# flexcompute/tidy3d

Hardware: AMD Instinct MI355X
Metric: Mcells/s on 512^3 Yee grid (higher is better)
Workload: dtype f32; 1 GPU; v0: vacuum, PEC walls, curl stencil only; 512^3 Yee cells, Ez point dipole (GaussianPulse 200 THz), random +-1e-3 initial fields; parallelism=z-slab x1, bytes_per_cell_step=72

## Files before the change

### tidy3d_amd/csrc/fdtd_fused2.hpp

```cpp
#pragma once
#include "fdtd_kernels.hpp"

namespace fdtd {

constexpr int kMaxInj = 256;
struct InjP {
  int n;
  const int* start;
  const int4* ent;
  const float* val;
  const float* val2;
  int e2_in_sweep;
  float* cap;
  const int* dstart;
  const int* dlist;
  const struct DumpBox* dboxes;
  float* dump;
};
struct DumpBox {
  int lo0, lo1, lo2, nx, ny, nz;
  int off[6];
};
constexpr int kMaxDumps = 8;
struct DampT {
// ... 93 lines not shown
        if (!fused2_instantiated(fused2_lb(W, opt), opt)) return false;
        const int rep = fused2_opt(nt, mat, mon, clip, damp, disp, src, wv, true, W);
        if (!clip && fused2_rep_word(opt) && !fused2_instantiated(fused2_lb(W, rep), rep)) return false;
      }
    }
  return true;
}
static_assert(fused2_words_instantiated(), "fused2_opt forms a word that no list of instantiations holds");

#if !defined(FDTD_NO_EXJ)
#define FDTD_NO_EXJ 0
#endif
constexpr bool fused2_exj(int lb, int opt) { return !FDTD_NO_EXJ && (opt & kF2Damp) == 0 && !(lb == 512 && (opt & kF2Mat) != 0); }
constexpr int fused2_xch_arrays(int lb, int opt) {
  const int wv = fused2_whatif(opt);
  if (wv) return wv == 13 ? 9 : ((wv >= 10 && wv <= 12) ? 6 + (wv == 11 ? 2 : 3) : 8);
  return fused2_exj(lb, opt) ? 9 : 8;
}
constexpr size_t fused2_lds_bytes(int lb, int opt, int waves) {
  return ((size_t)fused2_xch_arrays(lb, opt) * waves * 64 + ((opt & kF2Damp) ? 2 * 64 : 0)) * sizeof(float4) + ((opt & kF2Mat) ? (size_t)kMaxMedia * sizeof(float2) : 0);
}
static_assert(fused2_lds_bytes(1024, kF2NT | kF2Mat | kF2Mon | kF2Clip | kF2Disp | kF2Src, 16) <= 160 * 1024 && fused2_lds_bytes(1024, kF2Mat | kF2Damp, 16) <= 160 * 1024 &&
              2 * fused2_lds_bytes(512, kF2NT, 8) <= 160 * 1024 && 2 * fused2_lds_bytes(512, kF2Mat | kF2Damp, 8) <= 160 * 1024,
              "fused2_step_kernel: LDS of a workgroup (two per CU for eight waves)");
constexpr bool fused2_lds_pinned(int lb, int opt) {
  const int wv = fused2_whatif(opt), w = lb / 64;
  if (wv) return fused2_lds_bytes(lb, opt, 16) == ((size_t)(wv == 13 ? 9 : ((wv >= 10 && wv <= 12) ? 6 + (wv == 11 ? 2 : 3) : 8)) * 16 * 64) * sizeof(float4);
  return fused2_lds_bytes(lb, opt, w) == ((size_t)(fused2_exj(lb, opt) ? 9 : 8) * w * 64 + ((opt & 8) ? 2 * 64 : 0)) * sizeof(float4) + ((opt & 2) ? (size_t)kMaxMedia * sizeof(float2) : 0);
}
#define FDTD_F2_X(LBV, OV) && fused2_lds_pinned(LBV, OV)
static_assert(true FDTD_F2_LIST_ALL(FDTD_F2_X), "fused2_lds_bytes: the LDS of a listed instantiation changed");
#undef FDTD_F2_X
constexpr int kMaxCap = 1024;
constexpr int kSeamArrays = 13;

void launch_inject_values(hipStream_t st, float* val, const float* w_re, const float* w_im, const float2* wave,
                          long long step, int n);
struct Fused2Launch {
  hipStream_t st;
  int waves, opt, grid_blocks;
  GridP g; FieldP a, b; StepP s; MatP m;
  int zchunk, nbx, nby, nbz, xcd_remap;
  InjP inj; float* seam; DampT dmp; ClipP clip; TileClassP tcl; DispP dp; SrcP sr;
};
#define FDTD_F2_ARGS(L) (L).g, (L).a, (L).b, (L).s, (L).m, (L).zchunk, (L).nbx, (L).nby, (L).nbz, (L).xcd_remap, (L).inj, (L).seam, (L).dmp, (L).clip, (L).tcl, (L).dp, (L).sr
#define FDTD_F2_CASE(LBV, OV)                                                                                                      \
  case fused2_key(LBV, OV):                                                                                                        \
    hipLaunchKernelGGL((fused2_step_kernel<LBV, OV>), dim3(L.grid_blocks, 1, 1), dim3(64, L.waves, 1), fused2_lds_bytes(LBV, OV, L.waves), L.st, \
                       FDTD_F2_ARGS(L));                                                                                           \
    return true;
#define FDTD_F2_LAUNCHER(NAME, LIST)                                                                                               \
  bool NAME(const Fused2Launch& L) {                                                                                               \
    switch (fused2_key(fused2_lb(L.waves, L.opt), L.opt)) { LIST(FDTD_F2_CASE) default: return false; }                            \
  }
bool launch_fused2_step(const Fused2Launch& L);
bool launch_fused2_step_src(const Fused2Launch& L);
bool launch_fused2_step_whatif(const Fused2Launch& L);
bool launch_fused2_step_disp(const Fused2Launch& L);
bool launch_fused2_step_clip(const Fused2Launch& L);
void launch_inject_table(hipStream_t st, float* tab, long long stride, long long off, const float* w_re, const float* w_im,
                         const float2* wave, long long n_steps, int n);
constexpr int kPairMons = 4;
struct PairRecP {
  int n_mon;
  int pre_done;
  BoxP box[kPairMons];
  int nc[kPairMons];
  int comp[kPairMons][6];
  int cap_off[kPairMons];
  float* out_n[kPairMons];
  float* out_m[kPairMons];
};
void launch_pair_record(hipStream_t st, const PairRecP& r, long long max_cells, const GridP& g, const FieldP& a, const FieldP& b,
                        const float* cap);
struct DftDumpP { int n; int slot[3]; int off[3]; };
void launch_dft_record_dump(hipStream_t st, const DftDumpP& r, const float* dump, float2* acc, long long cells, long long fstride,
                            const float2* phase, int nf);
void launch_seams(hipStream_t st, const GridP& g, const FieldP& b, const StepP& s, const MatP& m, const float* seam,
                  int n_seams, const DampT& dmp, const ClipP& clip, const InjP& inj, const SrcP& sr = SrcP{}, float* rep = nullptr);
constexpr int kRepArraysHost = 7;
inline size_t seam_scratch_floats(const GridP& g, int n_tiles_x) { return (size_t)n_tiles_x * kSeamArrays * (size_t)(g.nz + 2) * (size_t)g.ny; }
inline size_t seam_rep_floats(const GridP& g, int n_tiles_x) { return (size_t)n_tiles_x * kRepArraysHost * (size_t)g.nz * (size_t)g.ny; }
void launch_seam_flush(hipStream_t st, const GridP& g, const FieldP& b, const float* rep, int n_seams);

}
```

### tidy3d_amd/csrc/fdtd_kernels2.hpp

```cpp
#pragma once
#include "fdtd_fused2.hpp"

namespace fdtd {

__global__ __launch_bounds__(256) void pair_record_kernel(PairRecP r, GridP g, FieldP a, FieldP b, const float* cap) {
  const int mi = blockIdx.y / 6, ic = blockIdx.y % 6;
  if (mi >= r.n_mon || ic >= r.nc[mi]) return;
  const BoxP bx = r.box[mi];
  const long long cells = (long long)bx.nx * bx.ny * bx.nz;
  const long long t = (long long)blockIdx.x * blockDim.x + threadIdx.x;
  if (t >= cells) return;
  const int c = r.comp[mi][ic];
  const int lx = (int)(t % bx.nx), ly = (int)((t / bx.nx) % bx.ny), lz = (int)(t / ((long long)bx.nx * bx.ny));
  const long long p = (long long)(bx.lo2 + lz) * g.sxy + (long long)(bx.lo1 + ly) * g.nx + bx.lo0 + lx;
  const long long idx = (long long)ic * cells + t;
  const float* fa = c == 0 ? a.ex : (c == 1 ? a.ey : (c == 2 ? a.ez : (c == 3 ? a.hx : (c == 4 ? a.hy : a.hz))));
  const float* fb = c == 0 ? b.ex : (c == 1 ? b.ey : (c == 2 ? b.ez : (c == 3 ? b.hx : (c == 4 ? b.hy : b.hz))));
  const float mid = cap[r.cap_off[mi] + idx];
  float* on = r.out_n[mi];
  float* om = r.out_m[mi];
  if (c < 3) {
    if (on && !r.pre_done) on[idx] = 1.0f * fa[p];
    if (om) om[idx] = 1.0f * mid;
  } else {
// ... 6 lines not shown
                                                              long long fstride, const float2* phase, int nf) {
  const int q = blockIdx.y;
  const long long t = (long long)blockIdx.x * blockDim.x + threadIdx.x;
  if (t >= cells || q >= r.n) return;
  const float v = dump[r.off[q] + t];
  float2* a0 = acc + (long long)r.slot[q] * cells;
  for (int k = 0; k < nf; ++k) {
    const float2 ph = phase[k];
    float2 a = a0[(long long)k * fstride + t];
    a.x += v * ph.x;
    a.y += v * ph.y;
    a0[(long long)k * fstride + t] = a;
  }
}

__global__ __launch_bounds__(256) void inject_table_kernel(float* tab, long long stride, long long off, const float* w_re,
                                                           const float* w_im, const float2* wave, long long n_steps, int n) {
  const long long g = (long long)blockIdx.x * blockDim.x + threadIdx.x;
  if (g >= n_steps * n) return;
  const long long step = g / n;
  const int t = (int)(g % n);
  const float2 a = wave[step];
  tab[step * stride + off + t] = w_re[t] * a.x - w_im[t] * a.y;
}

__global__ __launch_bounds__(256) void inject_values_kernel(float* val, const float* w_re, const float* w_im,
                                                            const float2* wave, long long step, int n) {
  const int t = threadIdx.x;
  if (t >= n) return;
  const float2 a = wave[step];
  val[t] = w_re[t] * a.x - w_im[t] * a.y;
}

__device__ __forceinline__ long long seam_at(const GridP& g, int seam, int arr, int j, int k) {
  return (((long long)seam * kSeamArrays + arr) * (g.nz + 2) + (k + 1)) * g.ny + j;
}

constexpr int kRepArrays = 7;
__device__ __forceinline__ long long rep_base(const GridP& g, int n_tiles_x) {
  return (long long)n_tiles_x * kSeamArrays * (g.nz + 2) * g.ny;
}
__device__ __forceinline__ long long rep_at(const GridP& g, int seam, int arr, int j, int k) {
  return (((long long)seam * kRepArrays + arr) * g.nz + k) * g.ny + j;
}

__device__ __forceinline__ float lane_next(float v) {
#if defined(__HIP_DEVICE_COMPILE__)
  const int x = __builtin_bit_cast(int, v);
  return __builtin_bit_cast(float, __builtin_amdgcn_update_dpp(x, x, 0x130, 0xf, 0xf, false));
#else
  return __shfl_down(v, 1);
#endif
}
__device__ __forceinline__ float lane_prev(float v) {
#if defined(__HIP_DEVICE_COMPILE__)
  const int x = __builtin_bit_cast(int, v);
  return __builtin_bit_cast(float, __builtin_amdgcn_update_dpp(x, x, 0x138, 0xf, 0xf, false));
#else
  return __shfl_up(v, 1);
#endif
}

__device__ __forceinline__ void lds_dma16(const float* base, unsigned off, float4* dst, int lane) {
#if defined(__HIP_DEVICE_COMPILE__)
  const unsigned lds_addr = __builtin_amdgcn_readfirstlane((unsigned)(size_t)dst);
  unsigned keep;
  asm volatile("s_mov_b32 %0, m0\n\ts_mov_b32 m0, %2\n\ts_nop 0\n\tglobal_load_lds_dwordx4 %1, %3\n\ts_mov_b32 m0, %0"
               : "=&s"(keep) : "v"(off), "s"(lds_addr), "s"(base) : "memory");
#else
  dst[lane] = *reinterpret_cast<const float4*>(reinterpret_cast<const char*>(base) + off);
#endif
}
__device__ __forceinline__ void lds_dma_wait() {
// ... 14 lines not shown
  return v;
}

__device__ __forceinline__ int lane_value(int v, int l) {
#if defined(__HIP_DEVICE_COMPILE__)
  return __builtin_amdgcn_readlane(v, l);
#else
  return __shfl(v, l);
#endif
}

template <int LB, int OPT>
__device__ __forceinline__ void fused2_step_tile(const GridP& g, const FieldP& a, const FieldP& b, const StepP& s, const MatP& m,
                                                 int zchunk, int nbx, int nby, int nbz, const InjP& inj,
                                                 float* __restrict__ seam, const DampT& dmp, const ClipP& clip, int t,
                                                 const DispP& dp, const SrcP& sr) {
  constexpr int V = 4;
  constexpr bool SRC = (OPT & kF2Src) != 0;
  constexpr bool NT = (OPT & kF2NT) != 0, MAT = (OPT & kF2Mat) != 0, MON = (OPT & kF2Mon) != 0;
  constexpr bool DISP = (OPT & kF2Disp) != 0;
  constexpr int WHATIF = fused2_whatif(OPT);
  constexpr int PF = (WHATIF >= 10 && WHATIF <= 12) ? WHATIF : 0;
  constexpr bool EZL = WHATIF == 15;
  constexpr bool EXJ = (WHATIF == 0 && (OPT & kF2NoExj) == 0) || WHATIF == 13 || EZL;
  constexpr bool E1S = PF != 0 || EZL;
  constexpr int XE = E1S ? 6 : 8, XZ = 7;
  [[maybe_unused]] constexpr int NPF = PF == 11 ? 2 : (PF ? 3 : 0);
  constexpr int NXCH = E1S ? 6 : 8;
  static_assert((!PF && !EZL) || (OPT & 0xff & ~kF2NT) == 0, "prefetch instantiations: the vacuum sweep only");
  constexpr bool DAMP = (OPT & kF2Damp) != 0;
  constexpr bool CLIP = (OPT & kF2Clip) != 0;
  constexpr bool REP = (OPT & kF2Rep) != 0;
  static_assert(!REP || (!CLIP && !PF && !EZL && !DISP && !SRC), "deferred seam repair: plain, materials and absorber sweeps of the whole grid");
  const bool per_x = CLIP && g.bcx0 == BC_PERIODIC;
  const int tile_y = t % nby;
  const int tile_x = (t / nby) % nbx;
  const int tile_z = t / (nby * nbx);
  HIP_DYNAMIC_SHARED(float4, xch)
  const int tx = threadIdx.x;
  const int ty = __builtin_amdgcn_readfirstlane((int)threadIdx.y);
  const int W = blockDim.y, R = W - 3;
  const int slot = W * 64;
  const int me = ty * 64 + tx;
  {
    const float4 z4 = {0.f, 0.f, 0.f, 0.f};
#pragma unroll
    for (int q = 0; q < NXCH; ++q) xch[q * slot + me] = z4;
  }
  [[maybe_unused]] float4* xdm = xch + (EXJ ? 9 : 8) * slot;
  [[maybe_unused]] float2* lut_s = reinterpret_cast<float2*>(xdm + (DAMP ? 2 * 64 : 0));
  if constexpr (MAT) {
    for (int q = me; q < m.n_media; q += slot) lut_s[q] = m.lut[q];
  }
  if constexpr (DAMP) {
    if (ty == 0) {
      const int ii = (tile_x * 64 + tx) * V;
      float4 b4 = {1.f, 1.f, 1.f, 1.f}, c4 = {1.f, 1.f, 1.f, 1.f};
      if (ii < g.nx) { b4 = *reinterpret_cast<const float4*>(dmp.fb[0] + ii); c4 = *reinterpret_cast<const float4*>(dmp.fc[0] + ii); }
      xdm[tx] = b4; xdm[64 + tx] = c4;
    }
  }
  __syncthreads();
  const float ca = m.ca1, cb = m.cb1;
  const int k0 = (CLIP ? clip.k0 : 0) + tile_z * zchunk;
  const int k1 = min(k0 + zchunk, CLIP ? clip.k1 : g.nz);
  const int kA = k0 > 0 ? k0 - 1 : 0;
// ... 74 lines not shown
    float ezx = lane_next(ezm[0]);
    if (act && (tx == 63 || last_x)) ezx = last_x ? (per_x ? a.ez[pb] : 0.f) : a.ez[pb + ux + V];
    const float ipz = s.ipz[kA - 1];
    ldf<V, true>(ho, uni(a.hx + pb), ubc);
    ldf<V, true>(hoy, uni(a.hy + pb), ubc);
    if constexpr (REP) {
      if (act && tx == 63 && !last_x) {
        const float* r = rpl + (long long)(kA - 1) * g.ny;
        hoy[V - 1] = r[0]; exm[V - 1] = r[2 * rep_arr]; eym[V - 1] = r[3 * rep_arr]; ezm[V - 1] = r[4 * rep_arr]; ezx = r[6 * rep_arr];
        if (use_jp) ezj[V - 1] = r[4 * rep_arr + 1];
      }
      if (xh) {
        const float* r = rpr + (long long)(kA - 1) * g.ny;
        eym[0] = r[5 * rep_arr]; ezm[0] = r[6 * rep_arr];
        if (use_jp) ezj[0] = r[6 * rep_arr + 1];
      }
    }
    if constexpr (DAMP) {
      const float czp = dmp.fc[2][kA - 1];
      const float4 b4 = xdm[tx], c4 = xdm[64 + tx];
      const float bx[V] = {b4.x, b4.y, b4.z, b4.w}, cx[V] = {c4.x, c4.y, c4.z, c4.w};
#pragma unroll
      for (int e = 0; e < V; ++e) { ho[e] *= bx[e] * cyv * czp; hoy[e] *= cx[e] * byv * czp; }
    }
#pragma unroll
    for (int e = 0; e < V; ++e) h1x[e] = upd_h(ho[e], ch, ezj[e] - ezm[e], ipy, eyk[e] - eym[e], ipz);
#pragma unroll
    for (int e = 0; e < V; ++e) {
      const float ez_ip = (e + 1 < V) ? ezm[(e + 1) % V] : ezx;
      h1y[e] = upd_h(hoy[e], ch, exk[e] - exm[e], ipz, ez_ip - ezm[e], ipx[e]);
    }
  }
  int cur = 0;
  const long long seam_arr = (long long)(g.nz + 2) * g.ny;
  const long long seam_row = seam_at(g, tile_x, 0, j, 0);
  struct Ld {
    float exn[V], eyn[V], ezk[V], exj[V], ezj[V], hxn[V], hyn[V], hzn[V];
    float eyx_g, ezx_g;
    float exn_m, ez_mm, ey_mm, ex_jm, hy_o, hz_o;
  };
  [[maybe_unused]] float4* pfb = xch + NXCH * slot;
  [[maybe_unused]] auto pf_issue = [&](int k) __attribute__((always_inline)) {
    if constexpr (PF != 0) {
      const long long pb = (long long)k * g.sxy + rowb;
      const long long up = (k < g.nz) ? g.sxy : 0;
      lds_dma_fence();
      if constexpr (PF == 10) {
        lds_dma16(uni(a.hx + pb), ubc, pfb + 0 * slot + ty * 64, tx);
        lds_dma16(uni(a.hy + pb), ubc, pfb + 1 * slot + ty * 64, tx);
        lds_dma16(uni(a.hz + pb), ubc, pfb + 2 * slot + ty * 64, tx);
      } else if constexpr (PF == 11) {
        lds_dma16(uni(a.ey + pb + up), ubc, pfb + 0 * slot + ty * 64, tx);
        lds_dma16(uni(a.hy + pb), ubc, pfb + 1 * slot + ty * 64, tx);
      } else {
        lds_dma16(uni(a.ex + pb + up), ubc, pfb + 0 * slot + ty * 64, tx);
        lds_dma16(uni(a.ey + pb + up), ubc, pfb + 1 * slot + ty * 64, tx);
        lds_dma16(uni(a.ez + pb), ubc, pfb + 2 * slot + ty * 64, tx);
      }
    }
  };
  [[maybe_unused]] auto pf_take = [&](int q, float (&o)[V]) __attribute__((always_inline)) {
    const float4 t4 = pfb[q * slot + me];
    o[0] = t4.x; o[1] = t4.y; o[2] = t4.z; o[3] = t4.w;
  };
  auto issue = [&](int k, Ld& L) __attribute__((always_inline)) {
    if constexpr (WHATIF == 3) {
      if (ty < 2 || ty == W - 1) {
        zero<V>(L.exn); zero<V>(L.eyn); zero<V>(L.ezk); zero<V>(L.exj); zero<V>(L.ezj); zero<V>(L.hxn); zero<V>(L.hyn); zero<V>(L.hzn);
// ... 59 lines not shown
          if (use_jp) {
            L.ezj[V - 1] = r[4 * rep_arr + 1];
            if (!EXJ || ty == W - 1 || k == kA) L.exj[V - 1] = r[2 * rep_arr + 1];
          }
        }
        if (xh) {
          const float* r = rpr + (long long)k * g.ny;
          L.ezk[0] = r[6 * rep_arr];
          if (up1) L.eyn[0] = r[5 * rep_arr + g.ny];
          if (use_jp) L.ezj[0] = r[6 * rep_arr + 1];
          if (do_e1) {
            L.exn_m = up1 ? r[2 * rep_arr + g.ny] : a.ex[pb + im + up];
            L.ez_mm = r[4 * rep_arr]; L.ey_mm = r[3 * rep_arr];
            if (use_jp) L.ex_jm = r[2 * rep_arr + 1];
            L.hy_o = r[0]; L.hz_o = r[rep_arr];
          }
        }
      }
    }
    if constexpr (PF != 0) {
      lds_dma_wait();
      if constexpr (PF == 10) { pf_take(0, L.hxn); pf_take(1, L.hyn); pf_take(2, L.hzn); }
      else if constexpr (PF == 11) { pf_take(0, L.eyn); pf_take(1, L.hyn); }
      else { pf_take(0, L.exn); pf_take(1, L.eyn); pf_take(2, L.ezk); }
    }
  };
  Ld LA, LB2;
  auto body = [&](int k, Ld& L) __attribute__((always_inline)) {
    const int txo = (MAT || DAMP) ? tx : opaque_lane(tx);
    const int i0o = (tile_x * 64 + txo) * V;
    const bool act = i0o < g.nx, last_x = i0o + V >= g.nx, first_x = i0o == 0;
    const bool xh = act && txo == 0 && (!first_x || per_x);
    [[maybe_unused]] const bool wall_x0 = first_x && !pmc_x0 && !per_x;
    const bool seam_l = (txo == 63 && !last_x) || (per_x && last_x), seam_r = txo == 0 && (tile_x > 0 || per_x);
    const long long seam_back = (tile_x > 0 ? -1 : (long long)(nbx - 1)) * kSeamArrays * seam_arr;
    const long long pb = (long long)k * g.sxy + rowb;
    const float ipz = s.ipz[k], idz = s.idz[k];
    [[maybe_unused]] float bzk = 1.f, czk = 1.f;
    if constexpr (DAMP) { bzk = dmp.fb[2][min(k, g.nz - 1)]; czk = dmp.fc[2][min(k, g.nz - 1)]; }
    int q0 = 0, q1 = 0;
    if (inj.n > 0) { q0 = inj.start[k]; q1 = inj.start[k + 1]; }
    [[maybe_unused]] int d0 = 0, d1 = 0;
    if constexpr (MON) { if (inj.dstart) { d0 = inj.dstart[k]; d1 = inj.dstart[k + 1]; } }
    float hy_m = 0.f, hz_m = 0.f;
    float (&exn)[V] = L.exn, (&eyn)[V] = L.eyn, (&ezk)[V] = L.ezk, (&exj)[V] = L.exj, (&ezj)[V] = L.ezj;
    float (&hxn)[V] = L.hxn, (&hyn)[V] = L.hyn, (&hzn)[V] = L.hzn;
    [[maybe_unused]] uint32_t rw = kBgWord;
    if constexpr (MAT) {
      if (do_e1) rw = m.roww[((long long)min(k, g.nz - 1) * g.ny + j) * nbx + tile_x];
    }
    [[maybe_unused]] int ss = -1;
    if constexpr (SRC) {
      if (do_e1 && k < g.nz) ss = sr.sseg[((long long)k * g.ny + j) * nbx + tile_x];
    }
    [[maybe_unused]] int ds = -1;
    if constexpr (DISP) {
      if (do_e1 && k < g.nz) ds = dp.dseg[((long long)k * g.ny + j) * nbx + tile_x];
    }
    if constexpr (WHATIF == 7) {
      issue(k, L);
      if (own && k > k0 && act) {
        const long long po = pb - g.sxy + i0;
        float o0[V], o1[V], o2[V];
#pragma unroll
        for (int e = 0; e < V; ++e) { o0[e] = L.exn[e] + L.exj[e]; o1[e] = L.ezk[e] + L.ezj[e]; o2[e] = L.eyn[e]; }
        stv_h<V, NT>(b.ex + po, o0); stv_h<V, NT>(b.ey + po, o2); stv_h<V, NT>(b.ez + po, o1);
        stv_h<V, NT>(b.hx + po, L.hxn); stv_h<V, NT>(b.hy + po, L.hyn); stv_h<V, NT>(b.hz + po, L.hzn);
      }
// ... 195 lines not shown
                  hit &= hit - 1;
                  const int d = lane_value(ev.x, l) - i0, c = lane_value(ev.z, l) - 8, w = lane_value(ev.w, l);
#pragma unroll
                  for (int e = 0; e < V; ++e)
                    if (d == e) inj.cap[w] = c == 0 ? e1xn[e] : (c == 1 ? e1yn[e] : e1zn[e]);
                }
              }
            }
          }
        }
        if constexpr (MON) {
          if (own && k >= k0 && k < k1) {
            for (int q = d0; q < d1; ++q) {
              const DumpBox bx = inj.dboxes[inj.dlist[q]];
              const int ly = j - bx.lo1, lz = k - bx.lo2;
              if (ly >= 0 && ly < bx.ny) {
                const long long rowo = ((long long)lz * bx.ny + ly) * bx.nx;
#pragma unroll
                for (int e = 0; e < V; ++e) {
                  const int lx = i0o + e - bx.lo0;
                  if (lx >= 0 && lx < bx.nx && act && (!CLIP || (i0o + e >= clip.i0 && i0o + e < clip.i1))) {
                    if (bx.off[0] >= 0) inj.dump[bx.off[0] + rowo + lx] = e1xn[e];
                    if (bx.off[1] >= 0) inj.dump[bx.off[1] + rowo + lx] = e1yn[e];
                    if (bx.off[2] >= 0) inj.dump[bx.off[2] + rowo + lx] = e1zn[e];
                    if (bx.off[3] >= 0) inj.dump[bx.off[3] + rowo + lx] = hxn[e];
                    if (bx.off[4] >= 0) inj.dump[bx.off[4] + rowo + lx] = hyn[e];
                    if (bx.off[5] >= 0) inj.dump[bx.off[5] + rowo + lx] = hzn[e];
                  }
                }
              }
            }
          }
        }
        if (WHATIF != 9 && (CLIP || (own && k >= k0 && k < k1)) && act) {
          float* sp = seam + seam_row + (long long)k * g.ny;
          if (seam_l) {
            sp[0] = hyn[V - 1];
            sp[seam_arr] = hzn[V - 1];
            sp[2 * seam_arr] = e1xn[V - 1];
            sp[3 * seam_arr] = e1yn[V - 1];
            sp[4 * seam_arr] = e1zn[V - 1];
          }
          if (seam_r) {
            sp[5 * seam_arr + seam_back] = e1yn[0];
            sp[6 * seam_arr + seam_back] = e1zn[0];
          }
        }
      }
    }
    float h2x[V], h2y[V], h2z[V];
    unspecified<V>(h2x); unspecified<V>(h2y); unspecified<V>(h2z);
    if (do_h2 && k > kA) {
      if constexpr (DAMP) {
        {
          const float4 b4 = xdm[tx];
          const float bx[V] = {b4.x, b4.y, b4.z, b4.w};
#pragma unroll
          for (int e = 0; e < V; ++e) h1x[e] *= bx[e] * cyv * cz_m;
        }
        {
          const float4 c4 = xdm[64 + tx];
          const float cx[V] = {c4.x, c4.y, c4.z, c4.w};
#pragma unroll
          for (int e = 0; e < V; ++e) { h1y[e] *= cx[e] * byv * cz_m; h1z[e] *= cx[e] * cyv * bz_m; }
        }
      }
      if constexpr (SRC) {
        if (ss_m >= 0 && act && sr.t->use_h2) {
          const long long qs = ((long long)ss_m * 3) * 256 + tx * V;
          float tx_[V], ty_[V], tz_[V];
          ldv<V>(tx_, sr.t->h2 + qs); ldv<V>(ty_, sr.t->h2 + qs + 256); ldv<V>(tz_, sr.t->h2 + qs + 512);
#pragma unroll
          for (int e = 0; e < V; ++e) { h1x[e] = h1x[e] + tx_[e]; h1y[e] = h1y[e] + ty_[e]; h1z[e] = h1z[e] + tz_[e]; }
          if (sr.t->h2b) {
            ldv<V>(tx_, sr.t->h2b + qs); ldv<V>(ty_, sr.t->h2b + qs + 256); ldv<V>(tz_, sr.t->h2b + qs + 512);
#pragma unroll
            for (int e = 0; e < V; ++e) { h1x[e] = h1x[e] + tx_[e]; h1y[e] = h1y[e] + ty_[e]; h1z[e] = h1z[e] + tz_[e]; }
          }
        }
// ... 9 lines not shown
              hit &= hit - 1;
              const int d = lane_value(ev.x, l) - i0o, code = lane_value(ev.z, l);
              const float v = inj.val2[lane_value(ev.w, l)];
#pragma unroll
              for (int e = 0; e < V; ++e) {
                const bool mine = d == e;
                h1x[e] = (mine && code == 3) ? h1x[e] + v : h1x[e];
                h1y[e] = (mine && code == 4) ? h1y[e] + v : h1y[e];
                h1z[e] = (mine && code == 5) ? h1z[e] + v : h1z[e];
              }
            }
          }
        }
      }
      float eyx = lane_next(e1y[0]);
      float ezx = lane_next(e1z[0]);
      if (txo == 63 || last_x) { eyx = 0.f; ezx = 0.f; }
      float4 t0, t1;
      if constexpr (WHATIF == 6) {
        t0 = make_float4(e1x[0], e1x[1], e1x[2], e1x[3]); t1 = make_float4(e1z[0], e1z[1], e1z[2], e1z[3]);
      } else {
        t0 = xch[(4 + (E1S ? 0 : (cur ^ 1) * 2) + 0) * slot + me + 64];
        t1 = xch[(4 + (E1S ? 0 : (cur ^ 1) * 2) + 1) * slot + me + 64];
      }
      const float exj1[V] = {t0.x, t0.y, t0.z, t0.w}, ezj1[V] = {t1.x, t1.y, t1.z, t1.w};
#pragma unroll
      for (int e = 0; e < V; ++e) {
        const float ey_ip = (e + 1 < V) ? e1y[(e + 1) % V] : eyx;
        const float ez_ip = (e + 1 < V) ? e1z[(e + 1) % V] : ezx;
        h2x[e] = upd_h(h1x[e], ch, ezj1[e] - e1z[e], ipy, e1yn[e] - e1y[e], ipz_m);
        h2y[e] = upd_h(h1y[e], ch, e1xn[e] - e1x[e], ipz_m, ez_ip - e1z[e], ipx[e]);
        h2z[e] = upd_h(h1z[e], ch, ey_ip - e1y[e], ipx[e], exj1[e] - e1x[e], ipy);
      }
      if constexpr (CLIP) {
        if (act) {
          float* sq = seam + seam_row + (long long)(k - 1) * g.ny;
          if (seam_l) {
            sq[7 * seam_arr] = h2x[V - 1];
            sq[8 * seam_arr] = h2y[V - 2];
            sq[9 * seam_arr] = h2z[V - 2];
          }
          if (seam_r) {
            sq[10 * seam_arr + seam_back] = h2x[0];
            sq[11 * seam_arr + seam_back] = h2y[0];
            sq[12 * seam_arr + seam_back] = h2z[0];
          }
        }
      }
    }
    if constexpr (WHATIF != 6) {
      float4 t4;
      if constexpr (!E1S) {
        t4.x = e1xn[0]; t4.y = e1xn[1]; t4.z = e1xn[2]; t4.w = e1xn[3];
        xch[(4 + cur * 2 + 0) * slot + me] = t4;
        t4.x = e1zn[0]; t4.y = e1zn[1]; t4.z = e1zn[2]; t4.w = e1zn[3];
        xch[(4 + cur * 2 + 1) * slot + me] = t4;
      }
      if constexpr (EXJ) {
        t4.x = exn[0]; t4.y = exn[1]; t4.z = exn[2]; t4.w = exn[3];
        xch[XE * slot + me] = t4;
      }
      if constexpr (EZL) {
        if (k + 1 <= k1) {
          t4.x = ezn_pre[0]; t4.y = ezn_pre[1]; t4.z = ezn_pre[2]; t4.w = ezn_pre[3];
          xch[XZ * slot + me] = t4;
        }
      }
      t4.x = h2x[0]; t4.y = h2x[1]; t4.z = h2x[2]; t4.w = h2x[3];
      xch[2 * slot + me] = t4;
      t4.x = h2z[0]; t4.y = h2z[1]; t4.z = h2z[2]; t4.w = h2z[3];
      xch[3 * slot + me] = t4;
    }
    if constexpr (WHATIF != 2 && WHATIF != 6 && WHATIF != 8) __syncthreads();
    if constexpr (E1S) {
      float4 t4;
      t4.x = e1xn[0]; t4.y = e1xn[1]; t4.z = e1xn[2]; t4.w = e1xn[3];
      xch[4 * slot + me] = t4;
      t4.x = e1zn[0]; t4.y = e1zn[1]; t4.z = e1zn[2]; t4.w = e1zn[3];
      xch[5 * slot + me] = t4;
// ... 76 lines not shown
          while (hit) {
            const int l = __ffsll(hit) - 1;
            hit &= hit - 1;
            const int d = lane_value(ev.x, l) - i0, code = lane_value(ev.z, l);
            const float v = inj.val2[lane_value(ev.w, l)];
#pragma unroll
            for (int e = 0; e < V; ++e) {
              if (d == e) {
                if (code == 0) ex[e] += v;
                else if (code == 1) ey[e] += v;
                else ez[e] += v;
              }
            }
          }
        }
      }
      if constexpr (DAMP) {
        if (dmp.e2) {
          {
            const float4 c4 = xdm[64 + tx];
            const float cx[V] = {c4.x, c4.y, c4.z, c4.w};
#pragma unroll
            for (int e = 0; e < V; ++e) ex[e] *= cx[e] * byv * bz_m;
          }
          {
            const float4 b4 = xdm[tx];
            const float bx[V] = {b4.x, b4.y, b4.z, b4.w};
#pragma unroll
            for (int e = 0; e < V; ++e) { ey[e] *= bx[e] * cyv * bz_m; ez[e] *= bx[e] * byv * cz_m; }
          }
        }
      }
      if (act && (!CLIP || (i0o >= clip.i0 && i0o < clip.i1))) {
        float* sq = seam + seam_row + (long long)(k - 1) * g.ny;
        if (!CLIP && WHATIF != 9 && txo == 63 && !last_x) {
          sq[7 * seam_arr] = h2x[V - 1];
          sq[8 * seam_arr] = h2y[V - 2];
          sq[9 * seam_arr] = h2z[V - 2];
        }
        if (!CLIP && WHATIF != 9 && txo == 0 && tile_x > 0) {
          sq[10 * seam_arr - kSeamArrays * seam_arr] = h2x[0];
          sq[11 * seam_arr - kSeamArrays * seam_arr] = h2y[0];
          sq[12 * seam_arr - kSeamArrays * seam_arr] = h2z[0];
        }
        const long long po = pb - g.sxy + i0;
        if (WHATIF != 5 || ex[0] == 3.0e38f) {
          stv_h<V, NT>(b.hx + po, h2x);
          stv_h<V, NT>(b.hy + po, h2y);
          stv_h<V, NT>(b.hz + po, h2z);
          stv_h<V, NT>(b.ex + po, ex);
          stv_h<V, NT>(b.ey + po, ey);
          stv_h<V, NT>(b.ez + po, ez);
        }
      }
    }
#pragma unroll
    for (int e = 0; e < V; ++e) {
      h2xm[e] = h2x[e]; h2ym[e] = h2y[e];
      h1x[e] = hxn[e]; h1y[e] = hyn[e]; h1z[e] = hzn[e];
      e1x[e] = e1xn[e]; e1y[e] = e1yn[e]; e1z[e] = e1zn[e];
      exk[e] = exn[e]; eyk[e] = eyn[e];
    }
    exk_m = L.exn_m;
    ipz_m = ipz; idz_m = idz;
    qm0 = q0; qm1 = q1;
    if constexpr (DAMP) { bz_m = bzk; cz_m = czk; }
    if constexpr (MAT) rw_m = rw;
    if constexpr (SRC) ss_m = ss;
    cur ^= 1;
  };
  if constexpr (PF != 0) pf_issue(kA);
  for (int k = kA; k <= k1; k += 2) {
    body(k, LA);
    if (k + 1 <= k1) body(k + 1, LB2);
  }
}

template <int LB, int OPT>
__device__ __forceinline__ void fused2_tile_by_class(const GridP& g, const FieldP& a, const FieldP& b, const StepP& s, const MatP& m,
                                                     int zchunk, int nbx, int nby, int nbz, const InjP& inj, float* __restrict__ seam,
                                                     const DampT& dmp, const ClipP& clip, int t, const DispP& dp, const SrcP& sr, const TileClassP& tcl) {
  if constexpr ((OPT & kF2Mat) != 0) {
    if (tcl.cls) {
      const int cl = tcl.cls[t] & 3;
      if (cl == 0) {
        fused2_step_tile<LB, (OPT & ~(kF2Mat | kF2Disp))>(g, a, b, s, m, zchunk, nbx, nby, nbz, inj, seam, dmp, clip, t, dp, sr);
// ... 24 lines not shown
    const int G = xcd_remap, full = total / (8 * G) * (8 * G);
    if (t < full) {
      const int x = t & 7, mloc = t >> 3;
      t = ((mloc / G) * 8 + x) * G + mloc % G;
    }
    if (t >= total) return;
  }
  constexpr int OPTK = OPT | (fused2_exj(LB, OPT) ? 0 : kF2NoExj);
  if constexpr ((OPT & kF2Src) != 0) {
    if (tcl.cls && !(tcl.cls[t] & 4)) {
      fused2_tile_by_class<LB, (OPTK & ~kF2Src)>(g, a, b, s, m, zchunk, nbx, nby, nbz, inj, seam, dmp, clip, t, dp, sr, tcl);
      return;
    }
  }
  fused2_tile_by_class<LB, OPTK>(g, a, b, s, m, zchunk, nbx, nby, nbz, inj, seam, dmp, clip, t, dp, sr, tcl);
}

__global__ __launch_bounds__(256) void seam_kernel(GridP g, FieldP b, StepP s, MatP m,
                                                   const float* __restrict__ seam, int n_seams, DampT dmp, ClipP clip, InjP inj, SrcP sr,
                                                   float* __restrict__ rep) {
  const long long t = (long long)blockIdx.x * blockDim.x + threadIdx.x;
  const int nj = clip.j1 - clip.j0;
  const long long per = (long long)nj * (clip.k1 - clip.k0);
  if (t >= per * n_seams) return;
  const int sm = (int)(t / per);
  const int k = clip.k0 + (int)((t % per) / nj), j = clip.j0 + (int)(t % nj);
  const bool wrap = g.bcx0 == BC_PERIODIC && sm == n_seams - 1;
  const int c = wrap ? g.nx : (sm + 1) * 256;
  const int cc = wrap ? 0 : c;
  const bool wl = c - 1 >= clip.i0 && c - 1 < clip.i1, wr = cc >= clip.i0 && cc < clip.i1;
  if (!wl && !wr) return;
  const float ch = g.ch;
  const float ipx = s.ipx[c - 1];
  auto A = [&](int a, int jj, int kk) { return seam[seam_at(g, sm, a, jj, kk)]; };
  auto h2 = [&](int jj, int kk, float& hy, float& hz) {
    const float e1x = A(2, jj, kk), e1y = A(3, jj, kk), e1z = A(4, jj, kk);
    const float e1x_jp = (jj + 1 < g.ny) ? A(2, jj + 1, kk) : 0.f;
    float h1y = A(0, jj, kk), h1z = A(1, jj, kk);
    if (dmp.fb[0]) {
      const float cxv = dmp.fc[0][c - 1];
      h1y *= cxv * dmp.fb[1][jj] * dmp.fc[2][kk];
      h1z *= cxv * dmp.fc[1][jj] * dmp.fb[2][kk];
    }
    if (sr.sseg && sr.t->use_h2) {
      const int blk = sr.sseg[((long long)kk * g.ny + jj) * ((g.nx + 255) >> 8) + ((c - 1) >> 8)];
      if (blk >= 0) {
        const long long qs = ((long long)blk * 3) * 256 + ((c - 1) & 255);
        h1y = h1y + sr.t->h2[qs + 256];
        h1z = h1z + sr.t->h2[qs + 512];
        if (sr.t->h2b) { h1y = h1y + sr.t->h2b[qs + 256]; h1z = h1z + sr.t->h2b[qs + 512]; }
      }
    }
    hy = upd_h(h1y, ch, A(2, jj, kk + 1) - e1x, s.ipz[kk], A(6, jj, kk) - e1z, ipx);
    hz = upd_h(h1z, ch, A(5, jj, kk) - e1y, ipx, e1x_jp - e1x, s.ipy[jj]);
  };
  float hy_m, hz_m;
  h2(j, k, hy_m, hz_m);
  const bool pmc_y0 = g.bcy0 == BC_PMC, pmc_z0 = !g.pec_z0;
  const bool wall_y = (j == 0) && !pmc_y0, wall_z = (k == 0) && !pmc_z0;
  const bool mir_y = (j == 0) && pmc_y0, mir_z = (k == 0) && pmc_z0;
  const long long pr = (long long)k * g.sxy + (long long)j * g.nx;
  const long long p = pr + cc, pl = pr + c - 1;
  if (!rep && wl) { b.hy[pl] = hy_m; b.hz[pl] = hz_m; }
  const float idy = s.idy[j], idz = s.idz[k], idx_m = s.idx[c - 1], idx_c = s.idx[cc];
  const float hx_m = A(7, j, k), hy_mm = A(8, j, k), hz_mm = A(9, j, k);
  const float hx_c = A(10, j, k), hy_c = A(11, j, k), hz_c = A(12, j, k);
  auto coef = [&](long long cell, int c) {
    return m.m4 ? m.lut[(m.m4[cell] >> (10 * c)) & 1023u] : make_float2(m.ca1, m.cb1);
  };
  float ex_m = 0.f, ey_m = 0.f, ez_m = 0.f, ey_c = 0.f, ez_c = 0.f;
  float hy_k = 0.f, hz_j = 0.f, dum;
  if (mir_z) hy_k = -hy_m; else if (!wall_z) h2(j, k - 1, hy_k, dum);
  if (mir_y) hz_j = -hz_m; else if (!wall_y) h2(j - 1, k, dum, hz_j);
  const float hxm_k = wall_z ? 0.f : (mir_z ? -hx_m : A(7, j, k - 1)), hxc_k = wall_z ? 0.f : (mir_z ? -hx_c : A(10, j, k - 1));
  const float hxm_j = wall_y ? 0.f : (mir_y ? -hx_m : A(7, j - 1, k)), hxc_j = wall_y ? 0.f : (mir_y ? -hx_c : A(10, j - 1, k));
  if (!wall_y && !wall_z) { const float2 q = coef(pl, 0); ex_m = upd_e(A(2, j, k), q.x, q.y, hz_m - hz_j, idy, hy_m - hy_k, idz); }
  if (!wall_z) {
    const float2 qm = coef(pl, 1), qc = coef(p, 1);
    ey_m = upd_e(A(3, j, k), qm.x, qm.y, hx_m - hxm_k, idz, hz_m - hz_mm, idx_m);
    ey_c = upd_e(A(5, j, k), qc.x, qc.y, hx_c - hxc_k, idz, hz_c - hz_m, idx_c);
  }
  if (!wall_y) {
    const float2 qm = coef(pl, 2), qc = coef(p, 2);
    ez_m = upd_e(A(4, j, k), qm.x, qm.y, hy_m - hy_mm, idx_m, hx_m - hxm_j, idy);
    ez_c = upd_e(A(6, j, k), qc.x, qc.y, hy_c - hy_m, idx_c, hx_c - hxc_j, idy);
  }
  if (sr.sseg && sr.t->use_e2) {
    const int nbxg = (g.nx + 255) >> 8;
    const int bl = sr.sseg[((long long)k * g.ny + j) * nbxg + ((c - 1) >> 8)], br = sr.sseg[((long long)k * g.ny + j) * nbxg + (cc >> 8)];
    if (bl >= 0) {
      const long long qs = ((long long)bl * 3) * 256 + ((c - 1) & 255);
      ex_m = ex_m + sr.t->e2[qs]; ey_m = ey_m + sr.t->e2[qs + 256]; ez_m = ez_m + sr.t->e2[qs + 512];
      if (sr.t->e2b) { ex_m = ex_m + sr.t->e2b[qs]; ey_m = ey_m + sr.t->e2b[qs + 256]; ez_m = ez_m + sr.t->e2b[qs + 512]; }
    }
    if (br >= 0) {
      const long long qs = ((long long)br * 3) * 256 + (cc & 255);
      ey_c = ey_c + sr.t->e2[qs + 256]; ez_c = ez_c + sr.t->e2[qs + 512];
      if (sr.t->e2b) { ey_c = ey_c + sr.t->e2b[qs + 256]; ez_c = ez_c + sr.t->e2b[qs + 512]; }
    }
  }
  if (inj.val2 && inj.e2_in_sweep) {
    const int q0 = inj.start[k], q1 = inj.start[k + 1];
    for (int q = q0; q < q1; ++q) {
      const int4 en = inj.ent[q];
      if (en.y != j || en.z >= 3) continue;
      const float v = inj.val2[en.w];
      if (en.x == c - 1) { if (en.z == 0) ex_m += v; else if (en.z == 1) ey_m += v; else ez_m += v; }
      else if (en.x == cc) { if (en.z == 1) ey_c += v; else if (en.z == 2) ez_c += v; }
    }
  }
  if (dmp.fb[0] && dmp.e2) {
    const float bxm = dmp.fb[0][c - 1], cxm = dmp.fc[0][c - 1], bxc = dmp.fb[0][cc];
    const float byv = dmp.fb[1][j], cyv = dmp.fc[1][j], bzv = dmp.fb[2][k], czv = dmp.fc[2][k];
    ex_m *= cxm * byv * bzv; ey_m *= bxm * cyv * bzv; ez_m *= bxm * byv * czv;
    ey_c *= bxc * cyv * bzv; ez_c *= bxc * byv * czv;
  }
  if (rep) {
    float* r = rep + rep_at(g, sm, 0, j, k);
// ... 22 lines not shown
```

Measured before the change: 206,600 Mcells/s.

## Pack seam scratch into per-cell 8-float records written with DPP lane gathers

The seam scratch changes from 13 separate planar arrays to interleaved 8-float records per (side, j, k). The h2 values are stored at row k instead of k-1. In the plain sweep, the boundary lanes now gather their values with DPP row shifts, so a few lanes write one contiguous record instead of many scattered single-float stores. The seam repair kernel reads the records back as float4 loads. This targets the scattered, uncoalesced seam traffic, at the cost of extra cross-lane ops in every lane and more complex indexing that could carry correctness risk.

Result: no change. 206,700 Mcells/s (median of 5 runs) (+0.1%).

```diff
diff --git a/tidy3d_amd/csrc/fdtd_fused2.hpp b/tidy3d_amd/csrc/fdtd_fused2.hpp
--- a/tidy3d_amd/csrc/fdtd_fused2.hpp
+++ b/tidy3d_amd/csrc/fdtd_fused2.hpp
@@ -149,7 +149,8 @@
 static_assert(true FDTD_F2_LIST_ALL(FDTD_F2_X), "fused2_lds_bytes: the LDS of a listed instantiation changed");
 #undef FDTD_F2_X
 constexpr int kMaxCap = 1024;
-constexpr int kSeamArrays = 13;
+constexpr int kSeamRec = 8, kSeamSides = 2;
+constexpr int kSeamL1 = 5, kSeamR1 = 2, kSeamRN = 5;
 
 void launch_inject_values(hipStream_t st, float* val, const float* w_re, const float* w_im, const float2* wave,
                           long long step, int n);
@@ -196,7 +197,7 @@
 void launch_seams(hipStream_t st, const GridP& g, const FieldP& b, const StepP& s, const MatP& m, const float* seam,
                   int n_seams, const DampT& dmp, const ClipP& clip, const InjP& inj, const SrcP& sr = SrcP{}, float* rep = nullptr);
 constexpr int kRepArraysHost = 7;
-inline size_t seam_scratch_floats(const GridP& g, int n_tiles_x) { return (size_t)n_tiles_x * kSeamArrays * (size_t)(g.nz + 2) * (size_t)g.ny; }
+inline size_t seam_scratch_floats(const GridP& g, int n_tiles_x) { return (size_t)n_tiles_x * kSeamSides * kSeamRec * (size_t)(g.nz + 2) * (size_t)g.ny; }
 inline size_t seam_rep_floats(const GridP& g, int n_tiles_x) { return (size_t)n_tiles_x * kRepArraysHost * (size_t)g.nz * (size_t)g.ny; }
 void launch_seam_flush(hipStream_t st, const GridP& g, const FieldP& b, const float* rep, int n_seams);
 
diff --git a/tidy3d_amd/csrc/fdtd_kernels2.hpp b/tidy3d_amd/csrc/fdtd_kernels2.hpp
--- a/tidy3d_amd/csrc/fdtd_kernels2.hpp
+++ b/tidy3d_amd/csrc/fdtd_kernels2.hpp
@@ -62,13 +62,54 @@
   val[t] = w_re[t] * a.x - w_im[t] * a.y;
 }
 
-__device__ __forceinline__ long long seam_at(const GridP& g, int seam, int arr, int j, int k) {
-  return (((long long)seam * kSeamArrays + arr) * (g.nz + 2) + (k + 1)) * g.ny + j;
+__device__ __forceinline__ long long seam_rec_at(const GridP& g, int seam, int side, int j, int k) {
+  return ((((long long)seam * kSeamSides + side) * (g.nz + 2) + (k + 1)) * g.ny + j) * kSeamRec;
+}
+
+template <int Q>
+__device__ __forceinline__ float row_from_above(float keep, float v, [[maybe_unused]] int lane) {
+#if defined(__HIP_DEVICE_COMPILE__)
+  return __builtin_bit_cast(float, __builtin_amdgcn_update_dpp(__builtin_bit_cast(int, keep), __builtin_bit_cast(int, v), 0x100 + Q, 0xf, 0xf, false));
+#else
+  const float t = __shfl(v, lane + Q);
+  return (lane & 15) + Q < 16 ? t : keep;
+#endif
+}
+template <int Q>
+__device__ __forceinline__ float row_from_below(float keep, float v, [[maybe_unused]] int lane) {
+#if defined(__HIP_DEVICE_COMPILE__)
+  return __builtin_bit_cast(float, __builtin_amdgcn_update_dpp(__builtin_bit_cast(int, keep), __builtin_bit_cast(int, v), 0x110 + Q, 0xf, 0xf, false));
+#else
+  const float t = __shfl(v, lane - Q);
+  return (lane & 15) >= Q ? t : keep;
+#endif
+}
+template <bool P1, bool P2>
+__device__ __forceinline__ void seam_put_left(float* sp, int lane, bool ok1, bool ok2, float v0, float v1, float v2, float v3, float v4,
+                                              float v5, float v6, float v7) {
+  float r = P1 ? v0 : v5;
+  if constexpr (P1) {
+    r = row_from_above<1>(r, v1, lane); r = row_from_above<2>(r, v2, lane); r = row_from_above<3>(r, v3, lane); r = row_from_above<4>(r, v4, lane);
+  }
+  if constexpr (P2) {
+    r = row_from_above<5>(r, v5, lane); r = row_from_above<6>(r, v6, lane); r = row_from_above<7>(r, v7, lane);
+  }
+  const int q = 63 - lane;
+  if (q < kSeamRec && (q < kSeamL1 ? (P1 && ok1) : (P2 && ok2))) sp[q] = r;
+}
+template <bool P1, bool P2>
+__device__ __forceinline__ void seam_put_right(float* sp, int lane, bool ok1, bool ok2, float v0, float v1, float v2, float v3, float v4) {
+  float r = P1 ? v0 : v2;
+  if constexpr (P1) r = row_from_below<1>(r, v1, lane);
+  if constexpr (P2) {
+    r = row_from_below<2>(r, v2, lane); r = row_from_below<3>(r, v3, lane); r = row_from_below<4>(r, v4, lane);
+  }
+  if (lane < kSeamRN && (lane < kSeamR1 ? (P1 && ok1) : (P2 && ok2))) sp[lane] = r;
 }
 
 constexpr int kRepArrays = 7;
 __device__ __forceinline__ long long rep_base(const GridP& g, int n_tiles_x) {
-  return (long long)n_tiles_x * kSeamArrays * (g.nz + 2) * g.ny;
+  return (long long)n_tiles_x * kSeamSides * kSeamRec * (g.nz + 2) * g.ny;
 }
 __device__ __forceinline__ long long rep_at(const GridP& g, int seam, int arr, int j, int k) {
   return (((long long)seam * kRepArrays + arr) * g.nz + k) * g.ny + j;
@@ -149,6 +190,7 @@
   constexpr bool CLIP = (OPT & kF2Clip) != 0;
   constexpr bool REP = (OPT & kF2Rep) != 0;
   static_assert(!REP || (!CLIP && !PF && !EZL && !DISP && !SRC), "deferred seam repair: plain, materials and absorber sweeps of the whole grid");
+  constexpr bool PACK = (OPT & (kF2Mat | kF2Mon | kF2Damp | kF2Clip | kF2Disp | kF2Src)) == 0 && WHATIF != 4 && WHATIF != 6 && WHATIF != 12;
   const bool per_x = CLIP && g.bcx0 == BC_PERIODIC;
   const int tile_y = t % nby;
   const int tile_x = (t / nby) % nbx;
@@ -289,8 +331,8 @@
     }
   }
   int cur = 0;
-  const long long seam_arr = (long long)(g.nz + 2) * g.ny;
-  const long long seam_row = seam_at(g, tile_x, 0, j, 0);
+  const long long seam_side = (long long)(g.nz + 2) * g.ny * kSeamRec;
+  const long long seam_row = seam_rec_at(g, tile_x, 0, j, 0);
   struct Ld {
     float exn[V], eyn[V], ezk[V], exj[V], ezj[V], hxn[V], hyn[V], hzn[V];
     float eyx_g, ezx_g;
@@ -416,8 +458,9 @@
     const bool act = i0o < g.nx, last_x = i0o + V >= g.nx, first_x = i0o == 0;
     const bool xh = act && txo == 0 && (!first_x || per_x);
     [[maybe_unused]] const bool wall_x0 = first_x && !pmc_x0 && !per_x;
-    const bool seam_l = (txo == 63 && !last_x) || (per_x && last_x), seam_r = txo == 0 && (tile_x > 0 || per_x);
-    const long long seam_back = (tile_x > 0 ? -1 : (long long)(nbx - 1)) * kSeamArrays * seam_arr;
+    const bool seam_l63 = (tile_x + 1) * 64 * V < g.nx, seam_lw = per_x && !seam_l63, seam_r0 = tile_x > 0 || per_x;
+    [[maybe_unused]] const bool seam_l = (txo == 63 && !last_x) || (per_x && last_x), seam_r = txo == 0 && seam_r0;
+    const long long seam_back = (1 + kSeamSides * (tile_x > 0 ? -1 : (long long)(nbx - 1))) * seam_side;
     const long long pb = (long long)k * g.sxy + rowb;
     const float ipz = s.ipz[k], idz = s.idz[k];
     [[maybe_unused]] float bzk = 1.f, czk = 1.f;
@@ -679,19 +722,10 @@
             }
           }
         }
-        if (WHATIF != 9 && (CLIP || (own && k >= k0 && k < k1)) && act) {
-          float* sp = seam + seam_row + (long long)k * g.ny;
-          if (seam_l) {
-            sp[0] = hyn[V - 1];
-            sp[seam_arr] = hzn[V - 1];
-            sp[2 * seam_arr] = e1xn[V - 1];
-            sp[3 * seam_arr] = e1yn[V - 1];
-            sp[4 * seam_arr] = e1zn[V - 1];
-          }
-          if (seam_r) {
-            sp[5 * seam_arr + seam_back] = e1yn[0];
-            sp[6 * seam_arr + seam_back] = e1zn[0];
-          }
+        if (!PACK && WHATIF != 9 && (CLIP || (own && k >= k0 && k < k1)) && act) {
+          float* sp = seam + seam_row + (long long)k * g.ny * kSeamRec;
+          if (seam_l) { sp[0] = hyn[V - 1]; sp[1] = hzn[V - 1]; sp[2] = e1xn[V - 1]; sp[3] = e1yn[V - 1]; sp[4] = e1zn[V - 1]; }
+          if (seam_r) { sp[seam_back] = e1yn[0]; sp[seam_back + 1] = e1zn[0]; }
         }
       }
     }
@@ -767,19 +801,11 @@
         h2y[e] = upd_h(h1y[e], ch, e1xn[e] - e1x[e], ipz_m, ez_ip - e1z[e], ipx[e]);
         h2z[e] = upd_h(h1z[e], ch, ey_ip - e1y[e], ipx[e], exj1[e] - e1x[e], ipy);
       }
-      if constexpr (CLIP) {
+      if constexpr (CLIP && !PACK) {
         if (act) {
-          float* sq = seam + seam_row + (long long)(k - 1) * g.ny;
-          if (seam_l) {
-            sq[7 * seam_arr] = h2x[V - 1];
-            sq[8 * seam_arr] = h2y[V - 2];
-            sq[9 * seam_arr] = h2z[V - 2];
-          }
-          if (seam_r) {
-            sq[10 * seam_arr + seam_back] = h2x[0];
-            sq[11 * seam_arr + seam_back] = h2y[0];
-            sq[12 * seam_arr + seam_back] = h2z[0];
-          }
+          float* sp = seam + seam_row + (long long)k * g.ny * kSeamRec;
+          if (seam_l) { sp[5] = h2x[V - 1]; sp[6] = h2y[V - 2]; sp[7] = h2z[V - 2]; }
+          if (seam_r) { sp[seam_back + 2] = h2x[0]; sp[seam_back + 3] = h2y[0]; sp[seam_back + 4] = h2z[0]; }
         }
       }
     }
@@ -922,16 +948,10 @@
         }
       }
       if (act && (!CLIP || (i0o >= clip.i0 && i0o < clip.i1))) {
-        float* sq = seam + seam_row + (long long)(k - 1) * g.ny;
-        if (!CLIP && WHATIF != 9 && txo == 63 && !last_x) {
-          sq[7 * seam_arr] = h2x[V - 1];
-          sq[8 * seam_arr] = h2y[V - 2];
-          sq[9 * seam_arr] = h2z[V - 2];
-        }
-        if (!CLIP && WHATIF != 9 && txo == 0 && tile_x > 0) {
-          sq[10 * seam_arr - kSeamArrays * seam_arr] = h2x[0];
-          sq[11 * seam_arr - kSeamArrays * seam_arr] = h2y[0];
-          sq[12 * seam_arr - kSeamArrays * seam_arr] = h2z[0];
+        if constexpr (!CLIP && !PACK && WHATIF != 9) {
+          float* sp = seam + seam_row + (long long)k * g.ny * kSeamRec;
+          if (seam_l) { sp[5] = h2x[V - 1]; sp[6] = h2y[V - 2]; sp[7] = h2z[V - 2]; }
+          if (seam_r) { sp[seam_back + 2] = h2x[0]; sp[seam_back + 3] = h2y[0]; sp[seam_back + 4] = h2z[0]; }
         }
         const long long po = pb - g.sxy + i0;
         if (WHATIF != 5 || ex[0] == 3.0e38f) {
@@ -942,6 +962,22 @@
           stv_h<V, NT>(b.ey + po, ey);
           stv_h<V, NT>(b.ez + po, ez);
         }
+      }
+    }
+    if constexpr (PACK && WHATIF != 9) {
+      const bool ok1 = CLIP ? do_e1 : (own && k >= k0 && k < k1);
+      const bool ok2 = CLIP ? (do_h2 && k > kA) : (own && k > k0);
+      if (ok1 || ok2) {
+        float* sp = seam + seam_row + (long long)k * g.ny * kSeamRec;
+        if (seam_l63) {
+          seam_put_left<true, true>(sp, txo, ok1, ok2, hyn[V - 1], hzn[V - 1], e1xn[V - 1], e1yn[V - 1], e1zn[V - 1], h2x[V - 1], h2y[V - 2], h2z[V - 2]);
+        } else if (seam_lw) {
+          if (act && last_x) {
+            if (ok1) { sp[0] = hyn[V - 1]; sp[1] = hzn[V - 1]; sp[2] = e1xn[V - 1]; sp[3] = e1yn[V - 1]; sp[4] = e1zn[V - 1]; }
+            if (ok2) { sp[5] = h2x[V - 1]; sp[6] = h2y[V - 2]; sp[7] = h2z[V - 2]; }
+          }
+        }
+        if (seam_r0) seam_put_right<true, true>(sp + seam_back, txo, ok1, ok2, e1yn[0], e1zn[0], h2x[0], h2y[0], h2z[0]);
       }
     }
 #pragma unroll
@@ -1032,11 +1068,15 @@
   if (!wl && !wr) return;
   const float ch = g.ch;
   const float ipx = s.ipx[c - 1];
-  auto A = [&](int a, int jj, int kk) { return seam[seam_at(g, sm, a, jj, kk)]; };
+  auto L0 = [&](int jj, int kk) { return *reinterpret_cast<const float4*>(seam + seam_rec_at(g, sm, 0, jj, kk)); };
+  auto L1 = [&](int jj, int kk) { return *reinterpret_cast<const float4*>(seam + seam_rec_at(g, sm, 0, jj, kk) + 4); };
+  auto R0 = [&](int jj, int kk) { return *reinterpret_cast<const float4*>(seam + seam_rec_at(g, sm, 1, jj, kk)); };
+  auto R1 = [&](int jj, int kk) { return seam[seam_rec_at(g, sm, 1, jj, kk) + 4]; };
   auto h2 = [&](int jj, int kk, float& hy, float& hz) {
-    const float e1x = A(2, jj, kk), e1y = A(3, jj, kk), e1z = A(4, jj, kk);
-    const float e1x_jp = (jj + 1 < g.ny) ? A(2, jj + 1, kk) : 0.f;
-    float h1y = A(0, jj, kk), h1z = A(1, jj, kk);
+    const float4 l0 = L0(jj, kk), r0 = R0(jj, kk);
+    const float e1x = l0.z, e1y = l0.w, e1z = L1(jj, kk).x;
+    const float e1x_jp = (jj + 1 < g.ny) ? L0(jj + 1, kk).z : 0.f;
+    float h1y = l0.x, h1z = l0.y;
     if (dmp.fb[0]) {
       const float cxv = dmp.fc[0][c - 1];
       h1y *= cxv * dmp.fb[1][jj] * dmp.fc[2][kk];
@@ -1051,8 +1091,8 @@
         if (sr.t->h2b) { h1y = h1y + sr.t->h2b[qs + 256]; h1z = h1z + sr.t->h2b[qs + 512]; }
       }
     }
-    hy = upd_h(h1y, ch, A(2, jj, kk + 1) - e1x, s.ipz[kk], A(6, jj, kk) - e1z, ipx);
-    hz = upd_h(h1z, ch, A(5, jj, kk) - e1y, ipx, e1x_jp - e1x, s.ipy[jj]);
+    hy = upd_h(h1y, ch, L0(jj, kk + 1).z - e1x, s.ipz[kk], r0.y - e1z, ipx);
+    hz = upd_h(h1z, ch, r0.x - e1y, ipx, e1x_jp - e1x, s.ipy[jj]);
   };
   float hy_m, hz_m;
   h2(j, k, hy_m, hz_m);
@@ -1063,8 +1103,9 @@
   const long long p = pr + cc, pl = pr + c - 1;
   if (!rep && wl) { b.hy[pl] = hy_m; b.hz[pl] = hz_m; }
   const float idy = s.idy[j], idz = s.idz[k], idx_m = s.idx[c - 1], idx_c = s.idx[cc];
-  const float hx_m = A(7, j, k), hy_mm = A(8, j, k), hz_mm = A(9, j, k);
-  const float hx_c = A(10, j, k), hy_c = A(11, j, k), hz_c = A(12, j, k);
+  const float4 lk = L0(j, k), lk1 = L1(j, k), rk = R0(j, k), lu1 = L1(j, k + 1), ru = R0(j, k + 1);
+  const float hx_m = lu1.y, hy_mm = lu1.z, hz_mm = lu1.w;
+  const float hx_c = ru.z, hy_c = ru.w, hz_c = R1(j, k + 1);
   auto coef = [&](long long cell, int c) {
     return m.m4 ? m.lut[(m.m4[cell] >> (10 * c)) & 1023u] : make_float2(m.ca1, m.cb1);
   };
@@ -1072,18 +1113,18 @@
   float hy_k = 0.f, hz_j = 0.f, dum;
   if (mir_z) hy_k = -hy_m; else if (!wall_z) h2(j, k - 1, hy_k, dum);
   if (mir_y) hz_j = -hz_m; else if (!wall_y) h2(j - 1, k, dum, hz_j);
-  const float hxm_k = wall_z ? 0.f : (mir_z ? -hx_m : A(7, j, k - 1)), hxc_k = wall_z ? 0.f : (mir_z ? -hx_c : A(10, j, k - 1));
-  const float hxm_j = wall_y ? 0.f : (mir_y ? -hx_m : A(7, j - 1, k)), hxc_j = wall_y ? 0.f : (mir_y ? -hx_c : A(10, j - 1, k));
-  if (!wall_y && !wall_z) { const float2 q = coef(pl, 0); ex_m = upd_e(A(2, j, k), q.x, q.y, hz_m - hz_j, idy, hy_m - hy_k, idz); }
+  const float hxm_k = wall_z ? 0.f : (mir_z ? -hx_m : lk1.y), hxc_k = wall_z ? 0.f : (mir_z ? -hx_c : rk.z);
+  const float hxm_j = wall_y ? 0.f : (mir_y ? -hx_m : L1(j - 1, k + 1).y), hxc_j = wall_y ? 0.f : (mir_y ? -hx_c : R0(j - 1, k + 1).z);
+  if (!wall_y && !wall_z) { const float2 q = coef(pl, 0); ex_m = upd_e(lk.z, q.x, q.y, hz_m - hz_j, idy, hy_m - hy_k, idz); }
   if (!wall_z) {
     const float2 qm = coef(pl, 1), qc = coef(p, 1);
-    ey_m = upd_e(A(3, j, k), qm.x, qm.y, hx_m - hxm_k, idz, hz_m - hz_mm, idx_m);
-    ey_c = upd_e(A(5, j, k), qc.x, qc.y, hx_c - hxc_k, idz, hz_c - hz_m, idx_c);
+    ey_m = upd_e(lk.w, qm.x, qm.y, hx_m - hxm_k, idz, hz_m - hz_mm, idx_m);
+    ey_c = upd_e(rk.x, qc.x, qc.y, hx_c - hxc_k, idz, hz_c - hz_m, idx_c);
   }
   if (!wall_y) {
     const float2 qm = coef(pl, 2), qc = coef(p, 2);
-    ez_m = upd_e(A(4, j, k), qm.x, qm.y, hy_m - hy_mm, idx_m, hx_m - hxm_j, idy);
-    ez_c = upd_e(A(6, j, k), qc.x, qc.y, hy_c - hy_m, idx_c, hx_c - hxc_j, idy);
+    ez_m = upd_e(lk1.x, qm.x, qm.y, hy_m - hy_mm, idx_m, hx_m - hxm_j, idy);
+    ez_c = upd_e(rk.y, qc.x, qc.y, hy_c - hy_m, idx_c, hx_c - hxc_j, idy);
   }
   if (sr.sseg && sr.t->use_e2) {
     const int nbxg = (g.nx + 255) >> 8;
```
